# stanford-iprl-lab/nerf_shared

Measured on AMD Instinct MI355X. Metric: rays_per_sec, higher is better.
Workload: dtype bf16; 1 GPU; lego_halfres_400x400_64c+128f_viewdirs_8x256_chunk4096; entry=Renderer.render(c2w=pose, retraw=False), chunk=4096, N_samples=64, N_importance=128, weights=random-init seeds 0/10, parallelism=single GPU

## Files before the change

nerf_shared_amd/csrc/render.hip:

```cpp
#include <hip/hip_runtime.h>
#include <cstring>
#include <math.h>

#include "kernels.h"
#include "launch_util.h"

namespace na {

constexpr int RAYS_PER_WG = 4;

constexpr size_t LDS_PER_CU = 160 * 1024;
static int pow2_at_least(int n) {
    int p = 2;
    while (p < n) p <<= 1;
    return p;
}
size_t composite_bwd_lds_bytes(int S) { return (size_t)RAYS_PER_WG * 3 * S * sizeof(float); }
size_t sample_pdf_lds_bytes(int n_bins) { return (size_t)RAYS_PER_WG * 2 * n_bins * sizeof(float); }
size_t resample_lds_bytes(int Nc, int Ni, bool with_composite) {
    return (size_t)RAYS_PER_WG * ((with_composite ? Nc : 0) + 2 * (size_t)(Nc - 1) + pow2_at_least(Nc) + pow2_at_least(Ni)) * sizeof(float);
}
static int reserve_lds(DynamicLdsOptIn &opt_in, const void *kernel, size_t bytes) {
    if (bytes > LDS_PER_CU) return NERF_AMD_EINVAL;
    if (bytes > 64 * 1024 && opt_in.ensure(kernel, LDS_PER_CU) != hipSuccess) return NERF_AMD_EHIP;
    return NERF_AMD_OK;
}

__device__ __forceinline__ void wave_lds_sync() {
    asm volatile("s_waitcnt lgkmcnt(0)" ::: "memory");
    __builtin_amdgcn_wave_barrier();
}

__device__ __forceinline__ double wave_incl_prod(double v, int lane) {
#pragma unroll
    for (int d = 1; d < 64; d <<= 1) {
        double o = __shfl_up(v, d);
        if (lane >= d) v *= o;
    }
    return v;
}
__device__ __forceinline__ double wave_incl_sum(double v, int lane) {
#pragma unroll
    for (int d = 1; d < 64; d <<= 1) {
        double o = __shfl_up(v, d);
        if (lane >= d) v += o;
    }
    return v;
}
template <class T>
__device__ __forceinline__ T wave_sum(T v) {
#pragma unroll
    for (int d = 32; d > 0; d >>= 1) v += __shfl_xor(v, d);
    return v;
}

__device__ __forceinline__ float z_of_t(float near, float far, float t, int lindisp) {
    if (!lindisp) return near * (1.0f - t) + far * t;
    return 1.0f / (1.0f / near * (1.0f - t) + 1.0f / far * t);
}

__global__ __launch_bounds__(256) void coarse_z_kernel(const float *rays, int ray_stride, const float *t_vals,
                                                       const float *t_rand, int64_t R, int Nc, int lindisp,
                                                       int perturb, float *z) {
    const int64_t total = R * Nc;
    for (int64_t i = (int64_t)blockIdx.x * blockDim.x + threadIdx.x; i < total; i += (int64_t)gridDim.x * blockDim.x) {
        const int64_t r = i / Nc;
        const int s = (int)(i - r * Nc);
        const float near = rays[r * ray_stride + 6], far = rays[r * ray_stride + 7];
        float zc = z_of_t(near, far, t_vals[s], lindisp);
        if (perturb) {
            float upper = zc, lower = zc;
            if (s + 1 < Nc) upper = 0.5f * (z_of_t(near, far, t_vals[s + 1], lindisp) + zc);
            if (s > 0) lower = 0.5f * (zc + z_of_t(near, far, t_vals[s - 1], lindisp));
            zc = lower + (upper - lower) * t_rand[i];
        }
        z[i] = zc;
    }
}

int launch_coarse_z(const float *rays, int ray_stride, const float *t_vals, const float *t_rand,
                    int64_t R, int Nc, int lindisp, int perturb, float *z, hipStream_t s) {
    if (R <= 0) return NERF_AMD_OK;
    int64_t blocks = (R * Nc + 255) / 256;
    if (blocks > 4096) blocks = 4096;
    hipLaunchKernelGGL(coarse_z_kernel, dim3((unsigned)blocks), dim3(256), 0, s, rays, ray_stride, t_vals, t_rand,
                       R, Nc, lindisp, perturb, z);
    return hipGetLastError() == hipSuccess ? NERF_AMD_OK : NERF_AMD_EHIP;
}

template <class StoreW>
__device__ __forceinline__ void composite_ray(const float *raw, int raw_ch, const float *z, const float *rays_d,
                                              int rays_d_stride, const float *noise, int64_t r, int S, int white_bkgd,
                                              float *rgb_map, float *disp_map, float *acc_map, float *depth_map, int lane,
                                              StoreW store_w) {
    const float *d = rays_d + r * rays_d_stride;
    const float dnorm = sqrtf(d[0] * d[0] + d[1] * d[1] + d[2] * d[2]);
    const float *zr = z + r * S;
    double carry = 1.0;
    float sr = 0.f, sg = 0.f, sb = 0.f, sdepth = 0.f, sacc = 0.f;
    for (int s0 = 0; s0 < S; s0 += 64) {
        const int s = s0 + lane;
        const bool in = s < S;
        float w = 0.f, zc = 0.f, cr = 0.f, cg = 0.f, cb = 0.f;
        double term = 1.0;
        float alpha = 0.f;
        if (in) {
            zc = zr[s];
            float dist = (s + 1 < S) ? zr[s + 1] - zc : 1e10f;
            dist = dist * dnorm;
            const float *q = raw + (r * S + s) * raw_ch;
            cr = 1.0f / (1.0f + expf(-q[0]));
            cg = 1.0f / (1.0f + expf(-q[1]));
            cb = 1.0f / (1.0f + expf(-q[2]));
            float sigma = q[3];
            if (noise) sigma = sigma + noise[r * S + s];
            sigma = fmaxf(sigma, 0.0f);
            alpha = 1.0f - expf(-sigma * dist);
            if (S == 1) alpha = 0.0f;
            term = (double)(1.0f - alpha + 1e-10f);
        }
        const double incl = wave_incl_prod(term, lane);
        double excl = __shfl_up(incl, 1);
        if (lane == 0) excl = 1.0;
        const float T = (float)(carry * excl);
        carry = carry * __shfl(incl, 63);
        if (in) {
            w = alpha * T;
            store_w(s, w);
        }
        sr += w * cr; sg += w * cg; sb += w * cb;
        sdepth += w * zc; sacc += w;
    }
    sr = wave_sum(sr); sg = wave_sum(sg); sb = wave_sum(sb);
    sdepth = wave_sum(sdepth); sacc = wave_sum(sacc);
    if (lane == 0) {
        if (white_bkgd) { const float bg = 1.0f - sacc; sr = sr + bg; sg = sg + bg; sb = sb + bg; }
        if (rgb_map) { rgb_map[3 * r] = sr; rgb_map[3 * r + 1] = sg; rgb_map[3 * r + 2] = sb; }
        if (depth_map) depth_map[r] = sdepth;
        if (acc_map) acc_map[r] = sacc;
        if (disp_map) {
            const float q = sdepth / sacc;
            const float m = (q != q) ? q : (q > 1e-10f ? q : 1e-10f);
            disp_map[r] = 1.0f / m;
        }
    }
}

__global__ __launch_bounds__(64 * RAYS_PER_WG) void composite_kernel(
    const float *raw, int raw_ch, const float *z, const float *rays_d, int rays_d_stride, const float *noise,
    int64_t R, int S, int white_bkgd, float *rgb_map, float *disp_map, float *acc_map, float *weights,
    float *depth_map) {
    const int lane = threadIdx.x & 63;
    const int64_t r = (int64_t)blockIdx.x * RAYS_PER_WG + (threadIdx.x >> 6);
    if (r >= R) return;
    composite_ray(raw, raw_ch, z, rays_d, rays_d_stride, noise, r, S, white_bkgd, rgb_map, disp_map, acc_map, depth_map, lane,
                  [&](int s, float w) { if (weights) weights[r * S + s] = w; });
}

int launch_composite(const float *raw, int raw_ch, const float *z, const float *rays_d, int rays_d_stride,
                     const float *noise, int64_t R, int S, int white_bkgd, float *rgb, float *disp, float *acc,
                     float *weights, float *depth, hipStream_t s) {
    if (R <= 0) return NERF_AMD_OK;
    if (S < 1 || raw_ch < 4) return NERF_AMD_EINVAL;
    const int64_t blocks = (R + RAYS_PER_WG - 1) / RAYS_PER_WG;
    hipLaunchKernelGGL(composite_kernel, dim3((unsigned)blocks), dim3(64 * RAYS_PER_WG), 0, s, raw, raw_ch, z,
                       rays_d, rays_d_stride, noise, R, S, white_bkgd, rgb, disp, acc, weights, depth);
    return hipGetLastError() == hipSuccess ? NERF_AMD_OK : NERF_AMD_EHIP;
}

__device__ __forceinline__ double wave_suffix_excl_sum(double v, int lane) {
    double incl = v;
#pragma unroll
    for (int d = 1; d < 64; d <<= 1) {
        double o = __shfl_down(incl, d);
        if (lane + d < 64) incl += o;
    }
    return incl - v;
}

__global__ __launch_bounds__(64 * RAYS_PER_WG) void composite_bwd_kernel(
    const float *raw, int raw_ch, const float *z, const float *rays_d, int rays_d_stride, const float *noise,
    int64_t R, int S, int white_bkgd, const float *g_rgb, const float *g_disp, const float *g_acc,
    const float *g_depth, const float *g_weights, float *g_raw, float *g_rays_d) {
    extern __shared__ float lds[];
    const int lane = threadIdx.x & 63, wv = threadIdx.x >> 6;
    const int64_t r = (int64_t)blockIdx.x * RAYS_PER_WG + wv;
    if (r >= R) return;
    float *sa = lds + wv * 3 * S, *sT = sa + S, *sw = sT + S;
    const float *d = rays_d + r * rays_d_stride;
    const float dnorm = sqrtf(d[0] * d[0] + d[1] * d[1] + d[2] * d[2]);
    const float *zr = z + r * S;
    double carry = 1.0;
    float sacc = 0.f, sdepth = 0.f;
    for (int s0 = 0; s0 < S; s0 += 64) {
        const int s = s0 + lane;
        const bool in = s < S;
        float alpha = 0.f, w = 0.f, zc = 0.f;
        double term = 1.0;
        if (in) {
            zc = zr[s];
            float dist = (s + 1 < S) ? zr[s + 1] - zc : 1e10f;
            dist = dist * dnorm;
            float sigma = raw[(r * S + s) * raw_ch + 3];
            if (noise) sigma = sigma + noise[r * S + s];
            sigma = fmaxf(sigma, 0.0f);
            alpha = 1.0f - expf(-sigma * dist);
            if (S == 1) alpha = 0.0f;
            term = (double)(1.0f - alpha + 1e-10f);
        }
        const double incl = wave_incl_prod(term, lane);
        double excl = __shfl_up(incl, 1);
        if (lane == 0) excl = 1.0;
        const float T = (float)(carry * excl);
        carry = carry * __shfl(incl, 63);
        if (in) {
            w = alpha * T;
            sa[s] = alpha; sT[s] = T; sw[s] = w;
        }
        sacc += w; sdepth += w * zc;
    }
    sacc = wave_sum(sacc); sdepth = wave_sum(sdepth);
    wave_lds_sync();
    const float gr = g_rgb ? g_rgb[3 * r] : 0.f, gg = g_rgb ? g_rgb[3 * r + 1] : 0.f, gb = g_rgb ? g_rgb[3 * r + 2] : 0.f;
    float gacc = g_acc ? g_acc[r] : 0.f, gdep = g_depth ? g_depth[r] : 0.f;
    if (g_disp) {
        const float q = sdepth / sacc;
        const float m = (q != q) ? q : (q > 1e-10f ? q : 1e-10f);
        const float gq = (q > 1e-10f || q != q) ? -g_disp[r] / (m * m) : 0.0f;
        gdep += gq / sacc;
        gacc += -gq * (q / sacc);
    }
    if (white_bkgd) gacc -= gr + gg + gb;
    double tail = 0.0;
    float gdn = 0.f;
    for (int s0 = ((S - 1) / 64) * 64; s0 >= 0; s0 -= 64) {
        const int s = s0 + lane;
        const bool in = s < S;
        float v = 0.f, w = 0.f, a = 0.f, T = 0.f, cr = 0.f, cg = 0.f, cb = 0.f, sig = 0.f, dz = 0.f, dist = 0.f;
        if (in) {
            const float *qv = raw + (r * S + s) * raw_ch;
            cr = 1.0f / (1.0f + expf(-qv[0]));
            cg = 1.0f / (1.0f + expf(-qv[1]));
            cb = 1.0f / (1.0f + expf(-qv[2]));
            sig = qv[3];
            if (noise) sig = sig + noise[r * S + s];
            const float zc = zr[s];
            dz = (s + 1 < S) ? zr[s + 1] - zc : 1e10f;
            dist = dz * dnorm;
            a = sa[s]; T = sT[s]; w = sw[s];
            v = gr * cr + gg * cg + gb * cb + gacc + gdep * zc;
            if (g_weights) v += g_weights[r * S + s];
        }
        const double u = (double)v * (double)w;
        const double later = wave_suffix_excl_sum(u, lane) + tail;
        tail += wave_sum(u);
        if (in) {
            float *o = g_raw + (r * S + s) * raw_ch;
            o[0] = gr * w * cr * (1.0f - cr);
            o[1] = gg * w * cg * (1.0f - cg);
            o[2] = gb * w * cb * (1.0f - cb);
            const float oma = 1.0f - a;
            const float e = expf(-fmaxf(sig, 0.0f) * dist);
            const float core = S > 1 ? e * (v * T - (float)later / (oma + 1e-10f)) : 0.0f;
            o[3] = sig > 0.0f ? dist * core : 0.0f;
            for (int c = 4; c < raw_ch; ++c) o[c] = 0.0f;
            gdn += core * fmaxf(sig, 0.0f) * dz;
        }
    }
    if (g_rays_d) {
        gdn = wave_sum(gdn);
        if (lane == 0) {
            g_rays_d[3 * r] = gdn * d[0] / dnorm;
            g_rays_d[3 * r + 1] = gdn * d[1] / dnorm;
            g_rays_d[3 * r + 2] = gdn * d[2] / dnorm;
        }
    }
}

int launch_composite_bwd(const float *raw, int raw_ch, const float *z, const float *rays_d, int rays_d_stride,
                         const float *noise, int64_t R, int S, int white_bkgd, const float *g_rgb, const float *g_disp,
                         const float *g_acc, const float *g_depth, const float *g_weights, float *g_raw, float *g_rays_d,
                         hipStream_t s) {
    if (R <= 0) return NERF_AMD_OK;
    if (S < 1 || raw_ch < 4) return NERF_AMD_EINVAL;
    const int64_t blocks = (R + RAYS_PER_WG - 1) / RAYS_PER_WG;
    const size_t lds = composite_bwd_lds_bytes(S);
    static DynamicLdsOptIn opt_in;
    if (int rc = reserve_lds(opt_in, reinterpret_cast<const void *>(composite_bwd_kernel), lds)) return rc;
    hipLaunchKernelGGL(composite_bwd_kernel, dim3((unsigned)blocks), dim3(64 * RAYS_PER_WG), lds, s, raw, raw_ch, z,
                       rays_d, rays_d_stride, noise, R, S, white_bkgd, g_rgb, g_disp, g_acc, g_depth, g_weights, g_raw,
                       g_rays_d);
    return hipGetLastError() == hipSuccess ? NERF_AMD_OK : NERF_AMD_EHIP;
}

template <class LoadW>
__device__ __forceinline__ void build_cdf(LoadW load_w, int nb, float *cdf, int lane) {
    double total = 0.0;
    for (int i0 = 0; i0 < nb - 1; i0 += 64) {
        const int i = i0 + lane;
        total += (i < nb - 1) ? (double)(load_w(i) + 1e-5f) : 0.0;
    }
    const float wsum = (float)wave_sum(total);
    double carry = 0.0;
    if (lane == 0) cdf[0] = 0.0f;
    for (int i0 = 0; i0 < nb - 1; i0 += 64) {
        const int i = i0 + lane;
        const float pdf = (i < nb - 1) ? (load_w(i) + 1e-5f) / wsum : 0.0f;
        const double incl = wave_incl_sum((double)pdf, lane);
        if (i < nb - 1) cdf[i + 1] = (float)(carry + incl);
        carry += __shfl(incl, 63);
    }
}

__device__ __forceinline__ float invert_cdf(const float *cdf, const float *bins, int nb, float u) {
    int lo = 0, hi = nb;
    while (lo < hi) {
        const int mid = (lo + hi) >> 1;
        if (cdf[mid] > u) hi = mid; else lo = mid + 1;
    }
    const int below = lo - 1 > 0 ? lo - 1 : 0;
    const int above = lo < nb - 1 ? lo : nb - 1;
    const float c0 = cdf[below], c1 = cdf[above];
    float denom = c1 - c0;
    if (denom < 1e-5f) denom = 1.0f;
    const float t = (u - c0) / denom;
    const float b0 = bins[below], b1 = bins[above];
    return b0 + t * (b1 - b0);
}

__global__ __launch_bounds__(64 * RAYS_PER_WG) void sample_pdf_kernel(const float *bins, const float *weights,
                                                                      const float *u, const float *t_lin, int64_t R,
                                                                      int nb, int N, float *samples) {
    extern __shared__ float lds[];
    const int lane = threadIdx.x & 63, wv = threadIdx.x >> 6;
    int64_t r = (int64_t)blockIdx.x * RAYS_PER_WG + wv;
    const bool live = r < R;
    if (!live) r = R - 1;
    float *cdf = lds + wv * 2 * nb, *bl = cdf + nb;
    const float *wr = weights + r * (nb - 1);
    build_cdf([&](int i) { return wr[i]; }, nb, cdf, lane);
    for (int i = lane; i < nb; i += 64) bl[i] = bins[r * nb + i];
    wave_lds_sync();
    if (!live) return;
    for (int i = lane; i < N; i += 64) {
        const float uu = u ? u[r * N + i] : t_lin[i];
        samples[r * N + i] = invert_cdf(cdf, bl, nb, uu);
    }
}

int launch_sample_pdf(const float *bins, const float *weights, const float *u, const float *t_lin,
                      int64_t R, int n_bins, int n_samples, float *samples, hipStream_t s) {
    if (R <= 0 || n_samples <= 0) return NERF_AMD_OK;
    if (n_bins < 2) return NERF_AMD_EINVAL;
    const int64_t blocks = (R + RAYS_PER_WG - 1) / RAYS_PER_WG;
    const size_t lds = sample_pdf_lds_bytes(n_bins);
    static DynamicLdsOptIn opt_in;
    if (int rc = reserve_lds(opt_in, reinterpret_cast<const void *>(sample_pdf_kernel), lds)) return rc;
    hipLaunchKernelGGL(sample_pdf_kernel, dim3((unsigned)blocks), dim3(64 * RAYS_PER_WG), lds, s, bins, weights, u,
                       t_lin, R, n_bins, n_samples, samples);
    return hipGetLastError() == hipSuccess ? NERF_AMD_OK : NERF_AMD_EHIP;
}

__device__ __forceinline__ unsigned order_key(float v) {
    const unsigned b = __builtin_bit_cast(unsigned, v);
    return (b & 0x80000000u) ? ~b : (b | 0x80000000u);
}

__device__ __forceinline__ bool wave_is_sorted(const float *x, int n, int lane) {
    bool ok = true;
    for (int i = lane; i + 1 < n; i += 64) ok = ok && order_key(x[i]) <= order_key(x[i + 1]);
    return __all(ok);
}

__device__ __forceinline__ void wave_bitonic_sort(float *x, int npad, int lane) {
    for (int k = 2; k <= npad; k <<= 1) {
        for (int j = k >> 1; j > 0; j >>= 1) {
            for (int t = lane; t < (npad >> 1); t += 64) {
                const int i = ((t & ~(j - 1)) << 1) | (t & (j - 1));
                const float a = x[i], b = x[i + j];
                const bool up = (i & k) == 0;
                if ((order_key(a) > order_key(b)) == up) { x[i] = b; x[i + j] = a; }
            }
            wave_lds_sync();
        }
    }
}

template <bool STRICT>
__device__ __forceinline__ int count_below(const float *x, int n, unsigned k) {
    int lo = 0, hi = n;
    while (lo < hi) {
        const int mid = (lo + hi) >> 1;
        const unsigned km = order_key(x[mid]);
        if (STRICT ? km < k : km <= k) lo = mid + 1; else hi = mid;
    }
    return lo;
}

template <class LoadW>
__device__ __forceinline__ void resample_ray(const float *z_coarse, LoadW load_w, const float *u, const float *t_lin,
                                             int64_t r, bool live, int Nc, int Ni, int pad_c, int pad_s, float *scratch,
                                             float *z_fine, float *z_std, int lane) {
    const int nb = Nc - 1;
    float *cdf = scratch, *bl = cdf + nb, *za = bl + nb, *zs = za + pad_c;
    const float *zr = z_coarse + r * Nc;
    build_cdf(load_w, nb, cdf, lane);
    for (int i = lane; i < nb; i += 64) bl[i] = 0.5f * (zr[i + 1] + zr[i]);
    for (int i = lane; i < pad_c; i += 64) za[i] = i < Nc ? zr[i] : INFINITY;
    for (int i = Ni + lane; i < pad_s; i += 64) zs[i] = INFINITY;
    wave_lds_sync();
    double sum = 0.0;
    for (int i = lane; i < Ni; i += 64) {
        const float uu = u ? u[r * Ni + i] : t_lin[i];
        const float v = invert_cdf(cdf, bl, nb, uu);
        zs[i] = v;
        sum += (double)v;
    }
    const double mean = wave_sum(sum) / (double)Ni;
    double ss = 0.0;
    for (int i = lane; i < Ni; i += 64) {
        const double dv = (double)zs[i] - mean;
        ss += dv * dv;
    }
    ss = wave_sum(ss);
    if (live && lane == 0 && z_std) z_std[r] = (float)sqrt(ss / (double)Ni);
    wave_lds_sync();
    if (!wave_is_sorted(zs, Ni, lane)) wave_bitonic_sort(zs, pad_s, lane);
    if (!wave_is_sorted(za, Nc, lane)) wave_bitonic_sort(za, pad_c, lane);
    if (!live) return;
    float *out = z_fine + r * (Nc + Ni);
    for (int i = lane; i < Nc; i += 64) {
        const float v = za[i];
        out[i + count_below<true>(zs, Ni, order_key(v))] = v;
    }
    for (int j = lane; j < Ni; j += 64) {
        const float v = zs[j];
        out[j + count_below<false>(za, Nc, order_key(v))] = v;
    }
}

__global__ __launch_bounds__(64 * RAYS_PER_WG) void resample_kernel(const float *z_coarse, const float *weights,
                                                                    const float *u, const float *t_lin, int64_t R,
                                                                    int Nc, int Ni, int pad_c, int pad_s, float *z_fine,
                                                                    float *z_std) {
    extern __shared__ float lds[];
    const int lane = threadIdx.x & 63, wv = threadIdx.x >> 6;
    int64_t r = (int64_t)blockIdx.x * RAYS_PER_WG + wv;
    const bool live = r < R;
    if (!live) r = R - 1;
    const float *wr = weights + r * Nc + 1;
    resample_ray(z_coarse, [&](int i) { return wr[i]; }, u, t_lin, r, live, Nc, Ni, pad_c, pad_s,
                 lds + wv * (2 * (Nc - 1) + pad_c + pad_s), z_fine, z_std, lane);
}

__global__ __launch_bounds__(64 * RAYS_PER_WG) void mid_stage_kernel(CompositeJob cj, ResampleJob rj, CompositeJob fj,
                                                                     int cr_blocks) {
    extern __shared__ float lds[];
    const int lane = threadIdx.x & 63, wv = threadIdx.x >> 6;
    if ((int)blockIdx.x < cr_blocks) {
        int64_t r = (int64_t)blockIdx.x * RAYS_PER_WG + wv;
        const bool live = r < cj.R;
        if (!live) r = cj.R - 1;
        const int Nc = cj.S;
        float *wl = lds + wv * (Nc + 2 * (Nc - 1) + rj.pad_c + rj.pad_s);
        composite_ray(cj.raw, cj.raw_ch, cj.z, cj.rays_d, cj.rays_d_stride, cj.noise, r, Nc, cj.white_bkgd,
                      live ? cj.rgb : nullptr, live ? cj.disp : nullptr, live ? cj.acc : nullptr, nullptr, lane,
                      [&](int s, float w) { wl[s] = w; if (live && cj.weights) cj.weights[r * Nc + s] = w; });
        wave_lds_sync();
        resample_ray(cj.z, [&](int i) { return wl[1 + i]; }, rj.u, rj.t_lin, r, live, Nc, rj.Ni, rj.pad_c, rj.pad_s,
                     wl + Nc, rj.z_fine, rj.z_std, lane);
    } else {
        const int64_t r = (int64_t)((int)blockIdx.x - cr_blocks) * RAYS_PER_WG + wv;
        if (r >= fj.R) return;
        composite_ray(fj.raw, fj.raw_ch, fj.z, fj.rays_d, fj.rays_d_stride, fj.noise, r, fj.S, fj.white_bkgd, fj.rgb, fj.disp,
                      fj.acc, nullptr, lane, [&](int s, float w) { if (fj.weights) fj.weights[r * fj.S + s] = w; });
    }
}

int launch_mid_stage(const CompositeJob &cj, const ResampleJob &rj, const CompositeJob *fj, hipStream_t s) {
    if (cj.R <= 0) return NERF_AMD_EINVAL;
    const int Nc = cj.S, Ni = rj.Ni;
    if (cj.raw_ch < 4 || Nc < 3 || Ni < 1) return NERF_AMD_EINVAL;
    ResampleJob r2 = rj;
    r2.pad_c = pow2_at_least(Nc); r2.pad_s = pow2_at_least(Ni);
    CompositeJob f2;
    std::memset(&f2, 0, sizeof(f2));
    if (fj) f2 = *fj;
    const int64_t cr_blocks = (cj.R + RAYS_PER_WG - 1) / RAYS_PER_WG;
    const int64_t f_blocks = (f2.R + RAYS_PER_WG - 1) / RAYS_PER_WG;
    if (cr_blocks + f_blocks >= ((int64_t)1 << 31)) return NERF_AMD_EINVAL;
    const size_t lds = resample_lds_bytes(Nc, Ni, true);
    static DynamicLdsOptIn opt_in;
    if (int rc = reserve_lds(opt_in, reinterpret_cast<const void *>(mid_stage_kernel), lds)) return rc;
    hipLaunchKernelGGL(mid_stage_kernel, dim3((unsigned)(cr_blocks + f_blocks)), dim3(64 * RAYS_PER_WG), lds, s, cj, r2, f2,
                       (int)cr_blocks);
    return hipGetLastError() == hipSuccess ? NERF_AMD_OK : NERF_AMD_EHIP;
}

int launch_resample(const float *z_coarse, const float *weights, const float *u, const float *t_lin,
                    int64_t R, int Nc, int Ni, float *z_fine, float *z_std, hipStream_t s) {
    if (R <= 0) return NERF_AMD_OK;
    if (Nc < 3 || Ni < 1) return NERF_AMD_EINVAL;
    const int pad_c = pow2_at_least(Nc), pad_s = pow2_at_least(Ni);
    const int64_t blocks = (R + RAYS_PER_WG - 1) / RAYS_PER_WG;
    const size_t lds = resample_lds_bytes(Nc, Ni, false);
    static DynamicLdsOptIn opt_in;
    if (int rc = reserve_lds(opt_in, reinterpret_cast<const void *>(resample_kernel), lds)) return rc;
    hipLaunchKernelGGL(resample_kernel, dim3((unsigned)blocks), dim3(64 * RAYS_PER_WG), lds, s, z_coarse, weights, u,
                       t_lin, R, Nc, Ni, pad_c, pad_s, z_fine, z_std);
    return hipGetLastError() == hipSuccess ? NERF_AMD_OK : NERF_AMD_EHIP;
}

__device__ __forceinline__ float norm3(float x, float y, float z) { return sqrtf((x * x + z * z) + y * y); }

struct RayGen {
    float fx, fy, cx, cy;
    float c2w[12], c2ws[12];
    int has_static, use_viewdirs, ndc, H, W;
    float near, far;
    float sx, sy;
};

__device__ __forceinline__ void cam_ray(const float *c, float dx, float dy, float dz, float *o, float *d) {
#pragma unroll
    for (int k = 0; k < 3; ++k) {
        d[k] = dx * c[4 * k] + dy * c[4 * k + 1] + dz * c[4 * k + 2];
        o[k] = c[4 * k + 3];
    }
}

__global__ __launch_bounds__(256) void make_rays_kernel(RayGen g, int64_t pix0, int64_t n, float *out) {
    const int64_t idx = (int64_t)blockIdx.x * blockDim.x + threadIdx.x;
    if (idx >= n) return;
    const int64_t pix = pix0 + idx;
    const float i = (float)(pix % g.W), j = (float)(pix / g.W);
    const float dx = (i - g.cx) / g.fx, dy = -(j - g.cy) / g.fy, dz = -1.0f;
    float o[3], d[3], vd[3];
    cam_ray(g.c2w, dx, dy, dz, o, d);
    vd[0] = d[0]; vd[1] = d[1]; vd[2] = d[2];
    if (g.has_static) cam_ray(g.c2ws, dx, dy, dz, o, d);
    const int ch = g.use_viewdirs ? 11 : 8;
    float *row = out + idx * ch;
    if (g.use_viewdirs) {
        const float nrm = norm3(vd[0], vd[1], vd[2]);
        row[8] = vd[0] / nrm; row[9] = vd[1] / nrm; row[10] = vd[2] / nrm;
    }
    if (g.ndc) {
        const float nearp = 1.0f;
        const float t = -(nearp + o[2]) / d[2];
        o[0] = o[0] + t * d[0]; o[1] = o[1] + t * d[1]; o[2] = o[2] + t * d[2];
        const float sx = g.sx, sy = g.sy;
        const float o0 = sx * o[0] / o[2], o1 = sy * o[1] / o[2], o2 = 1.0f + 2.0f * nearp / o[2];
        const float d0 = sx * (d[0] / d[2] - o[0] / o[2]);
        const float d1 = sy * (d[1] / d[2] - o[1] / o[2]);
        const float d2 = -2.0f * nearp / o[2];
        o[0] = o0; o[1] = o1; o[2] = o2; d[0] = d0; d[1] = d1; d[2] = d2;
    }
    row[0] = o[0]; row[1] = o[1]; row[2] = o[2];
    row[3] = d[0]; row[4] = d[1]; row[5] = d[2];
    row[6] = g.near; row[7] = g.far;
}

__global__ __launch_bounds__(256) void ndc_rays_kernel(float sx, float sy, float nearp, const float *ro, const float *rd,
                                                       int64_t n, float *oo, float *od) {
    const int64_t i = (int64_t)blockIdx.x * blockDim.x + threadIdx.x;
    if (i >= n) return;
    float o[3] = {ro[3 * i], ro[3 * i + 1], ro[3 * i + 2]};
    const float d[3] = {rd[3 * i], rd[3 * i + 1], rd[3 * i + 2]};
    const float t = -(nearp + o[2]) / d[2];
    o[0] = o[0] + t * d[0]; o[1] = o[1] + t * d[1]; o[2] = o[2] + t * d[2];
    oo[3 * i] = sx * o[0] / o[2];
    oo[3 * i + 1] = sy * o[1] / o[2];
    oo[3 * i + 2] = 1.0f + 2.0f * nearp / o[2];
    od[3 * i] = sx * (d[0] / d[2] - o[0] / o[2]);
    od[3 * i + 1] = sy * (d[1] / d[2] - o[1] / o[2]);
    od[3 * i + 2] = -2.0f * nearp / o[2];
}

__global__ __launch_bounds__(256) void ndc_rays_bwd_kernel(float sx, float sy, float nearp, const float *ro, const float *rd,
                                                           const float *g_oo, const float *g_od, int64_t n, float *g_ro,
                                                           float *g_rd) {
    const int64_t i = (int64_t)blockIdx.x * blockDim.x + threadIdx.x;
    if (i >= n) return;
    const float o[3] = {ro[3 * i], ro[3 * i + 1], ro[3 * i + 2]};
    const float d[3] = {rd[3 * i], rd[3 * i + 1], rd[3 * i + 2]};
    const float t = -(nearp + o[2]) / d[2];
    const float p[3] = {o[0] + t * d[0], o[1] + t * d[1], o[2] + t * d[2]};
    const float go[3] = {g_oo ? g_oo[3 * i] : 0.f, g_oo ? g_oo[3 * i + 1] : 0.f, g_oo ? g_oo[3 * i + 2] : 0.f};
    const float gd[3] = {g_od ? g_od[3 * i] : 0.f, g_od ? g_od[3 * i + 1] : 0.f, g_od ? g_od[3 * i + 2] : 0.f};
    const float ipz = 1.0f / p[2], idz = 1.0f / d[2];
    const float ax = sx * (go[0] - gd[0]), ay = sy * (go[1] - gd[1]);
    float gp[3];
    gp[0] = ax * ipz;
    gp[1] = ay * ipz;
    gp[2] = -(ax * p[0] + ay * p[1]) * ipz * ipz + 2.0f * nearp * ipz * ipz * (gd[2] - go[2]);
    float gdir[3];
    gdir[0] = sx * gd[0] * idz;
    gdir[1] = sy * gd[1] * idz;
    gdir[2] = -(sx * gd[0] * d[0] + sy * gd[1] * d[1]) * idz * idz;
    const float gt = gp[0] * d[0] + gp[1] * d[1] + gp[2] * d[2];
    float gor[3] = {gp[0], gp[1], gp[2]};
    gdir[0] += t * gp[0]; gdir[1] += t * gp[1]; gdir[2] += t * gp[2];
    gor[2] += -gt * idz;
    gdir[2] += -gt * t * idz;
    if (g_ro) { g_ro[3 * i] = gor[0]; g_ro[3 * i + 1] = gor[1]; g_ro[3 * i + 2] = gor[2]; }
    if (g_rd) { g_rd[3 * i] = gdir[0]; g_rd[3 * i + 1] = gdir[1]; g_rd[3 * i + 2] = gdir[2]; }
}

int launch_ndc_rays_bwd(int H, int W, double focal, float near, const float *rays_o, const float *rays_d, const float *g_oo,
                        const float *g_od, int64_t n, float *g_ro, float *g_rd, hipStream_t s) {
    if (n <= 0) return NERF_AMD_OK;
    const float sx = (float)(-1.0 / ((double)W / (2.0 * focal)));
    const float sy = (float)(-1.0 / ((double)H / (2.0 * focal)));
    hipLaunchKernelGGL(ndc_rays_bwd_kernel, dim3((unsigned)((n + 255) / 256)), dim3(256), 0, s, sx, sy, near, rays_o, rays_d,
                       g_oo, g_od, n, g_ro, g_rd);
    return hipGetLastError() == hipSuccess ? NERF_AMD_OK : NERF_AMD_EHIP;
}

int launch_ndc_rays(int H, int W, double focal, float near, const float *rays_o, const float *rays_d, int64_t n,
                    float *out_o, float *out_d, hipStream_t s) {
    if (n <= 0) return NERF_AMD_OK;
    const float sx = (float)(-1.0 / ((double)W / (2.0 * focal)));
    const float sy = (float)(-1.0 / ((double)H / (2.0 * focal)));
    hipLaunchKernelGGL(ndc_rays_kernel, dim3((unsigned)((n + 255) / 256)), dim3(256), 0, s, sx, sy, near, rays_o, rays_d,
                       n, out_o, out_d);
    return hipGetLastError() == hipSuccess ? NERF_AMD_OK : NERF_AMD_EHIP;
}

__global__ __launch_bounds__(256) void get_rays_bwd_kernel(RayGen g, int64_t pix0, int64_t n, const float *g_o,
                                                           const float *g_d, float *g_c2w) {
    float acc[12];
#pragma unroll
    for (int i = 0; i < 12; ++i) acc[i] = 0.f;
    for (int64_t idx = (int64_t)blockIdx.x * blockDim.x + threadIdx.x; idx < n; idx += (int64_t)gridDim.x * blockDim.x) {
        const int64_t pix = pix0 + idx;
        const float i = (float)(pix % g.W), j = (float)(pix / g.W);
        const float dir[3] = {(i - g.cx) / g.fx, -(j - g.cy) / g.fy, -1.0f};
#pragma unroll
        for (int k = 0; k < 3; ++k) {
            const float gd = g_d ? g_d[3 * idx + k] : 0.f;
#pragma unroll
            for (int m = 0; m < 3; ++m) acc[4 * k + m] += gd * dir[m];
            if (g_o) acc[4 * k + 3] += g_o[3 * idx + k];
        }
    }
#pragma unroll
    for (int i = 0; i < 12; ++i) {
        const float v = wave_sum(acc[i]);
        if ((threadIdx.x & 63) == 0) atomicAdd(g_c2w + i, v);
    }
}

int launch_get_rays_bwd(int H, int W, const double *K4, int64_t pix0, int64_t n, const float *g_o, const float *g_d,
                        float *g_c2w, hipStream_t s) {
    if (hipMemsetAsync(g_c2w, 0, 12 * sizeof(float), s) != hipSuccess) return NERF_AMD_EHIP;
    if (n <= 0) return NERF_AMD_OK;
    RayGen g;
    g.fx = (float)K4[0]; g.fy = (float)K4[1]; g.cx = (float)K4[2]; g.cy = (float)K4[3];
    g.H = H; g.W = W;
    int64_t blocks = (n + 255) / 256;
    if (blocks > 1024) blocks = 1024;
    hipLaunchKernelGGL(get_rays_bwd_kernel, dim3((unsigned)blocks), dim3(256), 0, s, g, pix0, n, g_o, g_d, g_c2w);
    return hipGetLastError() == hipSuccess ? NERF_AMD_OK : NERF_AMD_EHIP;
}

__device__ __forceinline__ unsigned quant8(float x) {
    const float c = fminf(fmaxf(x, 0.0f), 1.0f);
    return (unsigned)__fmul_rn(255.0f, c);
}

__global__ __launch_bounds__(256) void to8b_kernel(const float *x, int64_t n, uint8_t *out) {
    const int64_t n4 = n >> 2;
    const int64_t stride = (int64_t)gridDim.x * blockDim.x;
    for (int64_t i = (int64_t)blockIdx.x * blockDim.x + threadIdx.x; i < n4; i += stride) {
        const float4 v = reinterpret_cast<const float4 *>(x)[i];
        reinterpret_cast<unsigned *>(out)[i] = quant8(v.x) | (quant8(v.y) << 8) | (quant8(v.z) << 16) | (quant8(v.w) << 24);
    }
    const int64_t t = (n4 << 2) + (int64_t)blockIdx.x * blockDim.x + threadIdx.x;
    if (t < n) out[t] = (uint8_t)quant8(x[t]);
}

int launch_to8b(const float *x, int64_t n, uint8_t *out, hipStream_t s) {
    if (n <= 0) return NERF_AMD_OK;
    int64_t blocks = ((n >> 2) + 255) / 256;
    if (blocks < 1) blocks = 1;
    if (blocks > 256 * 16) blocks = 256 * 16;
    hipLaunchKernelGGL(to8b_kernel, dim3((unsigned)blocks), dim3(256), 0, s, x, n, out);
    return hipGetLastError() == hipSuccess ? NERF_AMD_OK : NERF_AMD_EHIP;
}

constexpr int MSE_BLOCK = 1024, MSE_PER_BLOCK = 16384, MSE_MAX_BLOCKS = 256;

constexpr int reduce_blocks(int64_t n, int per_block, int max_blocks) {
    const int64_t blocks = (n + per_block - 1) / per_block;
    return blocks < 1 ? 1 : blocks > max_blocks ? max_blocks : (int)blocks;
}
static_assert(reduce_blocks(1, 16384, 256) == 1 && reduce_blocks(16384, 16384, 256) == 1 && reduce_blocks(16385, 16384, 256) == 2,
              "one block up to 16384 values, two from 16385");
static_assert(reduce_blocks(256 * 16384, 16384, 256) == 256 && reduce_blocks(256 * 16384 + 1, 16384, 256) == 256 &&
              reduce_blocks((int64_t)1 << 40, 16384, 256) == 256, "clamped at the 256 rows of partials");
static_assert(IMG2MSE_EACH_MAX == MSE_PER_BLOCK && IMG2MSE_EACH_MAX == RAYS_AT_BWD_PER_BLOCK, "the batch limits are the one-block paths");

__device__ __forceinline__ float block_sum_1024(float v, float *part ) {
#pragma unroll
    for (int o = 32; o > 0; o >>= 1) v += __shfl_down(v, o, 64);
    if ((threadIdx.x & 63) == 0) part[threadIdx.x >> 6] = v;
    __syncthreads();
    float t = 0.f;
    if (threadIdx.x == 0)
#pragma unroll
        for (int k = 0; k < MSE_BLOCK / 64; ++k) t += part[k];
    return t;
}

__device__ __forceinline__ void img2mse_block(const float *x, const float *y, int64_t n, float *out, float *partials, int block,
                                              int n_blocks, float *part ) {
    float acc = 0.f;
    const int64_t stride = (int64_t)n_blocks * MSE_BLOCK;
    for (int64_t i = (int64_t)block * MSE_BLOCK + threadIdx.x; i < n; i += stride) {
        const float d = x[i] - y[i];
        acc += d * d;
    }
    const float t = block_sum_1024(acc, part);
    if (threadIdx.x == 0) {
        if (n_blocks == 1) out[0] = t / (float)n;
        else partials[block] = t;
    }
}

__global__ __launch_bounds__(MSE_BLOCK) void img2mse_kernel(const float *x, const float *y, int64_t y_stride, int64_t n, float *out,
                                                            float *partials) {
    __shared__ float part[MSE_BLOCK / 64];
    const int64_t b = blockIdx.y;
    img2mse_block(x + b * n, y + b * y_stride, n, out + b, partials, (int)blockIdx.x, (int)gridDim.x, part);
}

__global__ __launch_bounds__(MSE_MAX_BLOCKS) void img2mse_finish_kernel(const float *partials, int n_parts, int64_t n, float *out) {
    __shared__ float part[MSE_MAX_BLOCKS];
    part[threadIdx.x] = (int)threadIdx.x < n_parts ? partials[threadIdx.x] : 0.f;
    __syncthreads();
    if (threadIdx.x == 0) {
        float t = 0.f;
        for (int k = 0; k < n_parts; ++k) t += part[k];
        out[0] = t / (float)n;
    }
}

__device__ __forceinline__ void img2mse_bwd_body(const float *x, const float *y, int64_t n, const float *g, float *gx, float *gy) {
    const float s = g[0] * (2.0f / (float)n);
    const int64_t stride = (int64_t)gridDim.x * 256;
    for (int64_t i = (int64_t)blockIdx.x * 256 + threadIdx.x; i < n; i += stride) {
        const float v = s * (x[i] - y[i]);
        if (gx) gx[i] = v;
        if (gy) gy[i] = -v;
    }
}

__global__ __launch_bounds__(256) void img2mse_bwd_kernel(const float *x, const float *y, int64_t y_stride, int64_t n, const float *g,
                                                          float *gx, float *gy) {
    const int64_t b = blockIdx.y;
    img2mse_bwd_body(x + b * n, y + b * y_stride, n, g + b, gx ? gx + b * n : nullptr, gy ? gy + b * n : nullptr);
}

int launch_img2mse(const float *x, const float *y, int64_t y_stride, int64_t n, int B, float *out, float *partials, hipStream_t s) {
    if (B < 1 || B > POSE_BATCH_MAX || n < 1) return NERF_AMD_EINVAL;
    const int blocks = reduce_blocks(n, MSE_PER_BLOCK, MSE_MAX_BLOCKS);
    if (blocks > 1 && (!partials || B > 1)) return NERF_AMD_EINVAL;
    hipLaunchKernelGGL(img2mse_kernel, dim3((unsigned)blocks, (unsigned)B), dim3(MSE_BLOCK), 0, s, x, y, y_stride, n, out, partials);
    if (blocks > 1) hipLaunchKernelGGL(img2mse_finish_kernel, dim3(1), dim3(MSE_MAX_BLOCKS), 0, s, partials, blocks, n, out);
    return hipGetLastError() == hipSuccess ? NERF_AMD_OK : NERF_AMD_EHIP;
}

// ... 252 lines not shown
```

Baseline: 5.762 million rays/s.

## Use DPP/swizzle wave ops, register bitonic sort, branchless searches, vectorized coarse z

Replaces shfl-based wave scans and reductions with DPP, ds_swizzle, bpermute and readlane intrinsics. Adds a float4-vectorized coarse-z kernel that reuses neighbouring depth values across each quad of samples. Rewrites the CDF inversion and merge-rank binary searches as fixed-width branchless partition points that handle two queries per lane. Sorts up to 128 fine samples in registers with a DPP bitonic network and prefetches the first u values before compositing. The goal is to cut LDS traffic and divergence in the mid stage, in exchange for much more intricate lane-permutation code that carries a correctness risk.

```diff
diff --git a/nerf_shared_amd/csrc/render.hip b/nerf_shared_amd/csrc/render.hip
--- a/nerf_shared_amd/csrc/render.hip
+++ b/nerf_shared_amd/csrc/render.hip
@@ -31,10 +31,43 @@
     __builtin_amdgcn_wave_barrier();
 }
 
+template <int J>
+__device__ __forceinline__ int lane_xor_bits(int v, int lane) {
+    if constexpr (J == 1) return __builtin_amdgcn_update_dpp(0, v, 0xB1, 0xf, 0xf, true);
+    else if constexpr (J == 2) return __builtin_amdgcn_update_dpp(0, v, 0x4E, 0xf, 0xf, true);
+    else if constexpr (J == 8) return __builtin_amdgcn_update_dpp(0, v, 0x128, 0xf, 0xf, true);
+    else if constexpr (J == 4 || J == 16) return __builtin_amdgcn_ds_swizzle(v, 0x1F | (J << 10));
+    else return __builtin_amdgcn_ds_bpermute((lane ^ J) << 2, v);
+}
+__device__ __forceinline__ int lane_from_bits(int v, int src) { return __builtin_amdgcn_ds_bpermute(src << 2, v); }
+
+template <int J>
+__device__ __forceinline__ float lane_xor(float v, int lane) {
+    return __builtin_bit_cast(float, lane_xor_bits<J>(__builtin_bit_cast(int, v), lane));
+}
+template <int J>
+__device__ __forceinline__ unsigned lane_xor(unsigned v, int lane) { return (unsigned)lane_xor_bits<J>((int)v, lane); }
+template <int J>
+__device__ __forceinline__ double lane_xor(double v, int lane) {
+    const long long b = __builtin_bit_cast(long long, v);
+    const unsigned lo = (unsigned)lane_xor_bits<J>((int)b, lane), hi = (unsigned)lane_xor_bits<J>((int)(b >> 32), lane);
+    return __builtin_bit_cast(double, ((long long)hi << 32) | (long long)lo);
+}
+__device__ __forceinline__ double lane_from(double v, int src) {
+    const long long b = __builtin_bit_cast(long long, v);
+    const unsigned lo = (unsigned)lane_from_bits((int)b, src), hi = (unsigned)lane_from_bits((int)(b >> 32), src);
+    return __builtin_bit_cast(double, ((long long)hi << 32) | (long long)lo);
+}
+__device__ __forceinline__ double lane63(double v) {
+    const long long b = __builtin_bit_cast(long long, v);
+    const unsigned lo = (unsigned)__builtin_amdgcn_readlane((int)b, 63), hi = (unsigned)__builtin_amdgcn_readlane((int)(b >> 32), 63);
+    return __builtin_bit_cast(double, ((long long)hi << 32) | (long long)lo);
+}
+
 __device__ __forceinline__ double wave_incl_prod(double v, int lane) {
 #pragma unroll
     for (int d = 1; d < 64; d <<= 1) {
-        double o = __shfl_up(v, d);
+        double o = lane_from(v, lane - d);
         if (lane >= d) v *= o;
     }
     return v;
@@ -42,15 +75,16 @@
 __device__ __forceinline__ double wave_incl_sum(double v, int lane) {
 #pragma unroll
     for (int d = 1; d < 64; d <<= 1) {
-        double o = __shfl_up(v, d);
+        double o = lane_from(v, lane - d);
         if (lane >= d) v += o;
     }
     return v;
 }
 template <class T>
 __device__ __forceinline__ T wave_sum(T v) {
-#pragma unroll
-    for (int d = 32; d > 0; d >>= 1) v += __shfl_xor(v, d);
+    const int lane = (int)__lane_id();
+    v += lane_xor<32>(v, lane); v += lane_xor<16>(v, lane); v += lane_xor<8>(v, lane);
+    v += lane_xor<4>(v, lane); v += lane_xor<2>(v, lane); v += lane_xor<1>(v, lane);
     return v;
 }
 
@@ -78,9 +112,52 @@
     }
 }
 
+__global__ __launch_bounds__(256) void coarse_z_quad_kernel(const float *rays, int ray_stride, const float *t_vals,
+                                                            const float *t_rand, int64_t R, int Nc, int lindisp,
+                                                            int perturb, float *z) {
+    const int quads = Nc >> 2, rows = 256 / quads;
+    const int row = (int)threadIdx.x / quads, s0 = ((int)threadIdx.x - row * quads) * 4;
+    if (row >= rows) return;
+    float t[6];
+#pragma unroll
+    for (int k = 0; k < 6; ++k) t[k] = (s0 - 1 + k >= 0 && s0 - 1 + k < Nc) ? t_vals[s0 - 1 + k] : 0.0f;
+    for (int64_t r = (int64_t)blockIdx.x * rows + row; r < R; r += (int64_t)gridDim.x * rows) {
+        const float near = rays[r * ray_stride + 6], far = rays[r * ray_stride + 7];
+        float zt[6];
+#pragma unroll
+        for (int k = 0; k < 6; ++k) zt[k] = z_of_t(near, far, t[k], lindisp);
+        float4 o = make_float4(zt[1], zt[2], zt[3], zt[4]);
+        if (perturb) {
+            const float4 u = *reinterpret_cast<const float4 *>(t_rand + r * Nc + s0);
+            const float uu[4] = {u.x, u.y, u.z, u.w};
+            float res[4];
+#pragma unroll
+            for (int k = 0; k < 4; ++k) {
+                const int s = s0 + k;
+                const float zc = zt[k + 1];
+                float upper = zc, lower = zc;
+                if (s + 1 < Nc) upper = 0.5f * (zt[k + 2] + zc);
+                if (s > 0) lower = 0.5f * (zc + zt[k]);
+                res[k] = lower + (upper - lower) * uu[k];
+            }
+            o = make_float4(res[0], res[1], res[2], res[3]);
+        }
+        *reinterpret_cast<float4 *>(z + r * Nc + s0) = o;
+    }
+}
+
 int launch_coarse_z(const float *rays, int ray_stride, const float *t_vals, const float *t_rand,
                     int64_t R, int Nc, int lindisp, int perturb, float *z, hipStream_t s) {
     if (R <= 0) return NERF_AMD_OK;
+    const bool aligned = ((uintptr_t)z % 16 == 0) && (!perturb || (uintptr_t)t_rand % 16 == 0);
+    if (Nc % 4 == 0 && Nc <= 1024 && aligned) {
+        const int rows = 256 / (Nc >> 2);
+        int64_t blocks = (R + rows - 1) / rows;
+        if (blocks > 2048) blocks = 2048;
+        hipLaunchKernelGGL(coarse_z_quad_kernel, dim3((unsigned)blocks), dim3(256), 0, s, rays, ray_stride, t_vals, t_rand,
+                           R, Nc, lindisp, perturb, z);
+        return hipGetLastError() == hipSuccess ? NERF_AMD_OK : NERF_AMD_EHIP;
+    }
     int64_t blocks = (R * Nc + 255) / 256;
     if (blocks > 4096) blocks = 4096;
     hipLaunchKernelGGL(coarse_z_kernel, dim3((unsigned)blocks), dim3(256), 0, s, rays, ray_stride, t_vals, t_rand,
@@ -123,7 +200,7 @@
         double excl = __shfl_up(incl, 1);
         if (lane == 0) excl = 1.0;
         const float T = (float)(carry * excl);
-        carry = carry * __shfl(incl, 63);
+        carry = carry * lane63(incl);
         if (in) {
             w = alpha * T;
             store_w(s, w);
@@ -212,7 +289,7 @@
         double excl = __shfl_up(incl, 1);
         if (lane == 0) excl = 1.0;
         const float T = (float)(carry * excl);
-        carry = carry * __shfl(incl, 63);
+        carry = carry * lane63(incl);
         if (in) {
             w = alpha * T;
             sa[s] = alpha; sT[s] = T; sw[s] = w;
@@ -308,16 +385,39 @@
         const float pdf = (i < nb - 1) ? (load_w(i) + 1e-5f) / wsum : 0.0f;
         const double incl = wave_incl_sum((double)pdf, lane);
         if (i < nb - 1) cdf[i + 1] = (float)(carry + incl);
-        carry += __shfl(incl, 63);
-    }
-}
-
-__device__ __forceinline__ float invert_cdf(const float *cdf, const float *bins, int nb, float u) {
-    int lo = 0, hi = nb;
-    while (lo < hi) {
-        const int mid = (lo + hi) >> 1;
-        if (cdf[mid] > u) hi = mid; else lo = mid + 1;
-    }
+        carry += lane63(incl);
+    }
+}
+
+template <class Pred>
+__device__ __forceinline__ int partition_point(const float *x, int n, int P, Pred pred) {
+    int pos = 0;
+    for (int s = P >> 1; s > 0; s >>= 1) {
+        const int i = pos + s - 1;
+        const float xv = x[i];
+        if ((i < n) & pred(xv)) pos += s;
+    }
+    const float xv = x[pos < n ? pos : n - 1];
+    if ((pos < n) & pred(xv)) ++pos;
+    return pos;
+}
+
+template <class PredA, class PredB>
+__device__ __forceinline__ void partition_point2(const float *x, int n, int P, PredA pred_a, PredB pred_b, int &pa, int &pb) {
+    int a = 0, b = 0;
+    for (int s = P >> 1; s > 0; s >>= 1) {
+        const int ia = a + s - 1, ib = b + s - 1;
+        const float xa = x[ia], xb = x[ib];
+        if ((ia < n) & pred_a(xa)) a += s;
+        if ((ib < n) & pred_b(xb)) b += s;
+    }
+    const float xa = x[a < n ? a : n - 1], xb = x[b < n ? b : n - 1];
+    if ((a < n) & pred_a(xa)) ++a;
+    if ((b < n) & pred_b(xb)) ++b;
+    pa = a; pb = b;
+}
+
+__device__ __forceinline__ float sample_of_bin(const float *cdf, const float *bins, int nb, float u, int lo) {
     const int below = lo - 1 > 0 ? lo - 1 : 0;
     const int above = lo < nb - 1 ? lo : nb - 1;
     const float c0 = cdf[below], c1 = cdf[above];
@@ -326,6 +426,16 @@
     const float t = (u - c0) / denom;
     const float b0 = bins[below], b1 = bins[above];
     return b0 + t * (b1 - b0);
+}
+__device__ __forceinline__ int cdf_search_width(int nb) { return 1 << (32 - __clz(nb - 1)); }
+__device__ __forceinline__ float invert_cdf(const float *cdf, const float *bins, int nb, float u) {
+    return sample_of_bin(cdf, bins, nb, u, partition_point(cdf, nb, cdf_search_width(nb), [&](float c) { return !(c > u); }));
+}
+__device__ __forceinline__ void invert_cdf2(const float *cdf, const float *bins, int nb, float ua, float ub, float &va, float &vb) {
+    int la, lb;
+    partition_point2(cdf, nb, cdf_search_width(nb), [&](float c) { return !(c > ua); }, [&](float c) { return !(c > ub); }, la, lb);
+    va = sample_of_bin(cdf, bins, nb, ua, la);
+    vb = sample_of_bin(cdf, bins, nb, ub, lb);
 }
 
 __global__ __launch_bounds__(64 * RAYS_PER_WG) void sample_pdf_kernel(const float *bins, const float *weights,
@@ -386,19 +496,79 @@
     }
 }
 
-template <bool STRICT>
-__device__ __forceinline__ int count_below(const float *x, int n, unsigned k) {
-    int lo = 0, hi = n;
-    while (lo < hi) {
-        const int mid = (lo + hi) >> 1;
-        const unsigned km = order_key(x[mid]);
-        if (STRICT ? km < k : km <= k) lo = mid + 1; else hi = mid;
-    }
-    return lo;
+__device__ __forceinline__ float key_value(unsigned k) {
+    return __builtin_bit_cast(float, (k & 0x80000000u) ? (k ^ 0x80000000u) : ~k);
+}
+
+template <bool DPP, int E, class Other>
+__device__ __forceinline__ void wave_exchange(unsigned (&k)[E], bool low, Other other) {
+#pragma unroll
+    for (int e = 0; e < E; ++e) {
+        const unsigned o = other(k[e]);
+        if constexpr (DPP) {
+            const unsigned mn = k[e] < o ? k[e] : o, mx = k[e] < o ? o : k[e];
+            k[e] = low ? mn : mx;
+        } else {
+            k[e] = ((k[e] < o) == low) ? k[e] : o;
+        }
+    }
+}
+template <int J, int E>
+__device__ __forceinline__ void wave_clean(unsigned (&k)[E], int lane) {
+    wave_exchange<J == 1 || J == 2 || J == 8>(k, (lane & J) == 0, [&](unsigned v) { return lane_xor<J>(v, lane); });
+}
+
+template <int E>
+__device__ __forceinline__ void wave_sort_keys(unsigned (&k)[E], int lane) {
+    static_assert(E == 1 || E == 2, "one or two keys per lane");
+    wave_clean<1>(k, lane);
+    wave_exchange<true>(k, (lane & 2) == 0, [&](unsigned v) { return (unsigned)__builtin_amdgcn_update_dpp(0, (int)v, 0x1B, 0xf, 0xf, true); });
+    wave_clean<1>(k, lane);
+    wave_exchange<true>(k, (lane & 4) == 0, [&](unsigned v) { return (unsigned)__builtin_amdgcn_update_dpp(0, (int)v, 0x141, 0xf, 0xf, true); });
+    wave_clean<2>(k, lane); wave_clean<1>(k, lane);
+    wave_exchange<true>(k, (lane & 8) == 0, [&](unsigned v) { return (unsigned)__builtin_amdgcn_update_dpp(0, (int)v, 0x140, 0xf, 0xf, true); });
+    wave_clean<4>(k, lane); wave_clean<2>(k, lane); wave_clean<1>(k, lane);
+    wave_exchange<false>(k, (lane & 16) == 0, [&](unsigned v) { return (unsigned)__builtin_amdgcn_ds_swizzle((int)v, 0x7C1F); });
+    wave_clean<8>(k, lane); wave_clean<4>(k, lane); wave_clean<2>(k, lane); wave_clean<1>(k, lane);
+    wave_exchange<false>(k, (lane & 32) == 0, [&](unsigned v) { return (unsigned)lane_from_bits((int)v, lane ^ 63); });
+    wave_clean<16>(k, lane); wave_clean<8>(k, lane); wave_clean<4>(k, lane); wave_clean<2>(k, lane); wave_clean<1>(k, lane);
+    if constexpr (E == 2) {
+        const unsigned o0 = (unsigned)lane_from_bits((int)k[1], lane ^ 63), o1 = (unsigned)lane_from_bits((int)k[0], lane ^ 63);
+        k[0] = k[0] < o0 ? k[0] : o0;
+        k[1] = k[1] < o1 ? o1 : k[1];
+        wave_clean<32>(k, lane); wave_clean<16>(k, lane); wave_clean<8>(k, lane); wave_clean<4>(k, lane); wave_clean<2>(k, lane);
+        wave_clean<1>(k, lane);
+    }
+}
+template <int E>
+__device__ __forceinline__ void wave_sort_in_registers(float *x, int n, int lane) {
+    unsigned k[E];
+#pragma unroll
+    for (int e = 0; e < E; ++e) k[e] = order_key(e * 64 + lane < n ? x[e * 64 + lane] : INFINITY);
+    wave_sort_keys<E>(k, lane);
+#pragma unroll
+    for (int e = 0; e < E; ++e)
+        if (e * 64 + lane < n) x[e * 64 + lane] = key_value(k[e]);
+    wave_lds_sync();
+}
+
+__device__ __forceinline__ int count_below(const float *x, int n, int P, unsigned k) {
+    return partition_point(x, n, P, [&](float v) { return order_key(v) < k; });
+}
+
+__device__ __forceinline__ float load_u(const float *u, const float *t_lin, int64_t r, int Ni, int i) {
+    return u ? u[r * Ni + i] : t_lin[i];
+}
+struct FirstU { float a, b; };
+__device__ __forceinline__ FirstU load_first_u(const float *u, const float *t_lin, int64_t r, int Ni, int lane) {
+    FirstU f;
+    f.a = lane < Ni ? load_u(u, t_lin, r, Ni, lane) : 0.0f;
+    f.b = lane + 64 < Ni ? load_u(u, t_lin, r, Ni, lane + 64) : 0.0f;
+    return f;
 }
 
 template <class LoadW>
-__device__ __forceinline__ void resample_ray(const float *z_coarse, LoadW load_w, const float *u, const float *t_lin,
+__device__ __forceinline__ void resample_ray(const float *z_coarse, LoadW load_w, const float *u, const float *t_lin, FirstU u_first,
                                              int64_t r, bool live, int Nc, int Ni, int pad_c, int pad_s, float *scratch,
                                              float *z_fine, float *z_std, int lane) {
     const int nb = Nc - 1;
@@ -410,11 +580,14 @@
     for (int i = Ni + lane; i < pad_s; i += 64) zs[i] = INFINITY;
     wave_lds_sync();
     double sum = 0.0;
-    for (int i = lane; i < Ni; i += 64) {
-        const float uu = u ? u[r * Ni + i] : t_lin[i];
-        const float v = invert_cdf(cdf, bl, nb, uu);
-        zs[i] = v;
-        sum += (double)v;
+    for (int i0 = 0; i0 < Ni; i0 += 128) {
+        const int i = i0 + lane, j = i + 64;
+        float ua = u_first.a, ub = u_first.b;
+        if (i0 > 0) { ua = i < Ni ? load_u(u, t_lin, r, Ni, i) : 0.0f; ub = j < Ni ? load_u(u, t_lin, r, Ni, j) : 0.0f; }
+        float va, vb;
+        invert_cdf2(cdf, bl, nb, ua, ub, va, vb);
+        if (i < Ni) { zs[i] = va; sum += (double)va; }
+        if (j < Ni) { zs[j] = vb; sum += (double)vb; }
     }
     const double mean = wave_sum(sum) / (double)Ni;
     double ss = 0.0;
@@ -425,17 +598,26 @@
     ss = wave_sum(ss);
     if (live && lane == 0 && z_std) z_std[r] = (float)sqrt(ss / (double)Ni);
     wave_lds_sync();
-    if (!wave_is_sorted(zs, Ni, lane)) wave_bitonic_sort(zs, pad_s, lane);
+    if (!wave_is_sorted(zs, Ni, lane)) {
+        if (Ni <= 64) wave_sort_in_registers<1>(zs, Ni, lane);
+        else if (Ni <= 128) wave_sort_in_registers<2>(zs, Ni, lane);
+        else wave_bitonic_sort(zs, pad_s, lane);
+    }
     if (!wave_is_sorted(za, Nc, lane)) wave_bitonic_sort(za, pad_c, lane);
     if (!live) return;
     float *out = z_fine + r * (Nc + Ni);
     for (int i = lane; i < Nc; i += 64) {
         const float v = za[i];
-        out[i + count_below<true>(zs, Ni, order_key(v))] = v;
-    }
-    for (int j = lane; j < Ni; j += 64) {
-        const float v = zs[j];
-        out[j + count_below<false>(za, Nc, order_key(v))] = v;
+        out[i + count_below(zs, Ni, pad_s, order_key(v))] = v;
+    }
+    for (int j0 = 0; j0 < Ni; j0 += 128) {
+        const int i = j0 + lane, j = i + 64;
+        const float va = i < Ni ? zs[i] : INFINITY, vb = j < Ni ? zs[j] : INFINITY;
+        const unsigned ka = order_key(va), kb = order_key(vb);
+        int ca, cb;
+        partition_point2(za, Nc, pad_c, [&](float v) { return order_key(v) <= ka; }, [&](float v) { return order_key(v) <= kb; }, ca, cb);
+        if (i < Ni) out[i + ca] = va;
+        if (j < Ni) out[j + cb] = vb;
     }
 }
 
@@ -449,7 +631,7 @@
     const bool live = r < R;
     if (!live) r = R - 1;
     const float *wr = weights + r * Nc + 1;
-    resample_ray(z_coarse, [&](int i) { return wr[i]; }, u, t_lin, r, live, Nc, Ni, pad_c, pad_s,
+    resample_ray(z_coarse, [&](int i) { return wr[i]; }, u, t_lin, load_first_u(u, t_lin, r, Ni, lane), r, live, Nc, Ni, pad_c, pad_s,
                  lds + wv * (2 * (Nc - 1) + pad_c + pad_s), z_fine, z_std, lane);
 }
 
@@ -463,11 +645,12 @@
         if (!live) r = cj.R - 1;
         const int Nc = cj.S;
         float *wl = lds + wv * (Nc + 2 * (Nc - 1) + rj.pad_c + rj.pad_s);
+        const FirstU u_first = load_first_u(rj.u, rj.t_lin, r, rj.Ni, lane);
         composite_ray(cj.raw, cj.raw_ch, cj.z, cj.rays_d, cj.rays_d_stride, cj.noise, r, Nc, cj.white_bkgd,
                       live ? cj.rgb : nullptr, live ? cj.disp : nullptr, live ? cj.acc : nullptr, nullptr, lane,
                       [&](int s, float w) { wl[s] = w; if (live && cj.weights) cj.weights[r * Nc + s] = w; });
         wave_lds_sync();
-        resample_ray(cj.z, [&](int i) { return wl[1 + i]; }, rj.u, rj.t_lin, r, live, Nc, rj.Ni, rj.pad_c, rj.pad_s,
+        resample_ray(cj.z, [&](int i) { return wl[1 + i]; }, rj.u, rj.t_lin, u_first, r, live, Nc, rj.Ni, rj.pad_c, rj.pad_s,
                      wl + Nc, rj.z_fine, rj.z_std, lane);
     } else {
         const int64_t r = (int64_t)((int)blockIdx.x - cr_blocks) * RAYS_PER_WG + wv;
```

Result: no change. 5.789 million rays/s, median of 6 (+0.5%).
